# joeyee/Onet

Hardware: AMD Instinct MI355X
Metric: training images/sec (twin 256x256 pass) (higher is better)
Workload: dtype f32

## Files before the change

onet_amd/_lib.py:

```python
from __future__ import annotations

import ctypes
import os
import re

HERE = os.path.dirname(os.path.abspath(__file__))
HEADER = os.path.join(os.path.dirname(HERE), "include", "onet_hip.h")
LIBPATH = os.environ.get("ONET_HIP_LIB") or os.path.join(HERE, "libonet_hip.so")

_CT = {
    "int": ctypes.c_int,
    "int64_t": ctypes.c_int64,
    "uint64_t": ctypes.c_uint64,
    "float": ctypes.c_float,
    "double": ctypes.c_double,
}


def parse_header(path: str = HEADER):
    src = open(path).read()
    src = re.sub(r"/\*.*?\*/", " ", src, flags=re.S)
    src = re.sub(r"//[^\n]*", " ", src)
    src = re.sub(r"^\s*#.*$", " ", src, flags=re.M)
    protos = {}
    for m in re.finditer(r"((?:const\s+)?\w+\s*\*?)\s*(onet_\w+)\s*\(([^)]*)\)\s*;", src):
        ret, name, args = m.group(1).strip(), m.group(2), m.group(3).strip()
        if ret.endswith("*"):
            restype = ctypes.c_char_p if "char" in ret else ctypes.c_void_p
        else:
            restype = _CT[ret]
        argtypes, argnames = [], []
        if args and args != "void":
            for a in args.split(","):
                a = a.strip()
                mm = re.match(r"(?:const\s+)?(\w+)\s*(\*?)\s*(\w+)$", a)
                if not mm:
                    raise ValueError(f"cannot parse argument {a!r} of {name}")
                base, ptr, an = mm.groups()
                argtypes.append(ctypes.c_void_p if ptr else _CT[base])
                argnames.append(an)
        protos[name] = (restype, argtypes, argnames)
    return protos


class OnetHipError(RuntimeError):
    pass


_lib = None
_protos = None


def load(build_if_missing: bool = True):
    global _lib, _protos
    if _lib is not None:
        return _lib
    if not os.path.exists(LIBPATH):
        if not build_if_missing:
            raise OnetHipError(f"{LIBPATH} not built; run `python -m onet_amd.build`")
        from . import build as _build
        _build.build()
    lib = ctypes.CDLL(LIBPATH)
    _protos = parse_header()
    for name, (restype, argtypes, _) in _protos.items():
        try:
            fn = getattr(lib, name)
        except AttributeError as e:
            raise OnetHipError(f"libonet_hip.so does not export {name} declared in onet_hip.h") from e
        fn.restype = restype
        fn.argtypes = argtypes
    _lib = lib
    return lib


def last_error() -> str:
    return load().onet_last_error().decode()


PROFILE_HOOK = None


def call(name: str, *args, nbytes=None):
    lib = load()
    hook = PROFILE_HOOK
    tok = hook.begin() if hook is not None else None
    rc = getattr(lib, name)(*args)
    if tok is not None:
        hook.end(name, nbytes, tok)
    if rc != 0:
        raise OnetHipError(f"{name} failed ({rc}): {lib.onet_last_error().decode()}")
    return rc
```

onet_amd/build.py:

```python
import os
import subprocess
import sys

HERE = os.path.dirname(os.path.abspath(__file__))
CSRC = os.path.join(HERE, "csrc")
LIB = os.path.join(HERE, "libonet_hip.so")
SOURCES = ["abi.cpp", "conv_mfma.hip", "conv_wino4.hip", "conv_wino4w.hip", "conv_split.hip", "convt_gemm.hip", "stem.hip", "bn.hip", "spatial.hip", "head_loss.hip", "optim.hip", "evalside.hip", "clutter.hip"]
ARCH = "gfx950"


def _stale():
    if not os.path.exists(LIB):
        return True
    t = os.path.getmtime(LIB)
    deps = [os.path.join(CSRC, f) for f in os.listdir(CSRC) if f.endswith((".hip", ".cpp", ".hpp"))] + \
        [os.path.join(HERE, "..", "include", "onet_hip.h")]
    return any(os.path.getmtime(d) > t for d in deps)


def build(force=False, verbose=False, variant=None, flags=()):
    lib = LIB if variant is None else os.path.join(HERE, f"libonet_hip_{variant}.so")
    if variant is None and not force and not _stale():
        return LIB
    hipcc = os.environ.get("HIPCC", "/opt/rocm/bin/hipcc")
    objdir = CSRC if variant is None else os.path.join(CSRC, "_" + variant)
    os.makedirs(objdir, exist_ok=True)
    objs = []
    procs = []
    for src in SOURCES:
        obj = os.path.join(objdir, src.rsplit(".", 1)[0] + ".o")
        cmd = [hipcc, "-x", "hip", f"--offload-arch={ARCH}", "-O3", "-fPIC", "-std=c++17", "-Wall",
               "-Wno-unused-result", "-fno-slp-vectorize", *flags, "-c", os.path.join(CSRC, src), "-o", obj]
        if verbose:
            cmd.insert(-4, "-Rpass-analysis=kernel-resource-usage")
        procs.append((src, subprocess.Popen(cmd, stdout=subprocess.PIPE, stderr=subprocess.STDOUT, text=True)))
        objs.append(obj)
    failed = False
    for src, p in procs:
        out, _ = p.communicate()
        if p.returncode != 0:
            failed = True
            sys.stderr.write(f"[onet_amd.build] {src} failed:\n{out}\n")
        elif verbose or out.strip():
            sys.stderr.write(out)
    if failed:
        raise RuntimeError("hipcc failed building libonet_hip.so")
    subprocess.check_call([hipcc, "-shared", "-fPIC", f"--offload-arch={ARCH}", "-o", lib] + objs)
    return lib


if __name__ == "__main__":
    if "--variant" in sys.argv:
        i = sys.argv.index("--variant")
        print(build(variant=sys.argv[i + 1], flags=[a for a in sys.argv[i + 2:]]))
    else:
        print(build(force="--force" in sys.argv, verbose="-v" in sys.argv))
```

onet_amd/csrc/stem.hip:

```cpp
#include <algorithm>
#include "common.hpp"

using namespace onet;

namespace {

struct StemArgs {
    const float* x;
    int64_t x_bs;
    const float* w;
    float* z;
    int64_t z_bs;
    float* part;
    int B, Cout, H, W, tilesX, tilesY;
    int twin_B;
    float twin_bias;
};

constexpr int ST_TH = 16, ST_TW = 64, ST_LR = ST_TH + 2, ST_LC = ST_TW + 4;
constexpr int ST_MAXC = 128;

#define ONET_ST_DPP_ADD(v, ctrl, rmask) \
    v += __builtin_bit_cast(float, __builtin_amdgcn_update_dpp(0, __builtin_bit_cast(int, v), ctrl, rmask, 0xf, false))
__device__ __forceinline__ float wave_sum_hi(float v) {
    ONET_ST_DPP_ADD(v, 0x128, 0xf);
    ONET_ST_DPP_ADD(v, 0x124, 0xf);
    ONET_ST_DPP_ADD(v, 0x122, 0xf);
    ONET_ST_DPP_ADD(v, 0x121, 0xf);
    ONET_ST_DPP_ADD(v, 0x142, 0xa);
    ONET_ST_DPP_ADD(v, 0x143, 0xc);
    return v;
}
#undef ONET_ST_DPP_ADD

template <int CIN>
__global__ __launch_bounds__(256) void stem_conv_stats_kernel(StemArgs a) {
    __shared__ float tile[CIN][ST_LR][ST_LC];
    __shared__ float sc[4][ST_MAXC][2];
    int bid = blockIdx.x;
    const int tx = bid % a.tilesX;
    bid /= a.tilesX;
    const int ty = bid % a.tilesY;
    const int b = bid / a.tilesY;
    const int y0 = ty * ST_TH, x0 = tx * ST_TW;
    const int tid = threadIdx.x, lane = tid & 63, wid = tid >> 6;
    const int HW = a.H * a.W;
    const bool comp = a.twin_B > 0 && b >= a.twin_B;
    const float* xb = a.x + (int64_t)(comp ? b - a.twin_B : b) * a.x_bs;

    for (int i = tid; i < CIN * ST_LR * 66; i += 256) {
        const int ci = i / (ST_LR * 66), r = (i / 66) % ST_LR, c = i % 66;
        const int yy = y0 - 1 + r, xx = x0 - 1 + c;
        const bool ok = yy >= 0 && yy < a.H && xx >= 0 && xx < a.W;
        float v = ok ? xb[(int64_t)ci * HW + (int64_t)yy * a.W + xx] : 0.f;
        if (comp && ok) v = fminf(fmaxf(1.f - v + a.twin_bias, 0.f), 1.f);
        tile[ci][r][c] = v;
    }
    __syncthreads();

    const int r = tid >> 4, q = tid & 15;
    float win[CIN][3][6];
#pragma unroll
    for (int ci = 0; ci < CIN; ++ci)
#pragma unroll
        for (int dy = 0; dy < 3; ++dy)
#pragma unroll
            for (int dx = 0; dx < 6; ++dx) win[ci][dy][dx] = tile[ci][r + dy][4 * q + dx];

    float* zb = a.z + (int64_t)b * a.z_bs + (int64_t)(y0 + r) * a.W + x0 + 4 * q;
    for (int co = 0; co < a.Cout; ++co) {
        const float* wp = a.w + (int64_t)co * CIN * 9;
        float acc[4] = {0.f, 0.f, 0.f, 0.f};
#pragma unroll
        for (int ci = 0; ci < CIN; ++ci)
#pragma unroll
            for (int dy = 0; dy < 3; ++dy)
#pragma unroll
                for (int dx = 0; dx < 3; ++dx) {
                    const float wv = wp[(ci * 3 + dy) * 3 + dx];
#pragma unroll
                    for (int j = 0; j < 4; ++j) acc[j] = fmaf(wv, win[ci][dy][dx + j], acc[j]);
                }
        *reinterpret_cast<float4*>(zb + (int64_t)co * HW) = make_float4(acc[0], acc[1], acc[2], acc[3]);
        if (a.part) {
            const float pv = __builtin_bit_cast(float, __builtin_amdgcn_readfirstlane(__builtin_bit_cast(int, acc[0])));
            float s1 = 0.f, s2 = 0.f;
#pragma unroll
            for (int j = 0; j < 4; ++j) {
                const float d = acc[j] - pv;
                s1 += d;
                s2 = fmaf(d, d, s2);
            }
            s1 = wave_sum_hi(s1);
            s2 = wave_sum_hi(s2);
            if (lane == 63) {
                sc[wid][co][0] = fmaf(s1, 1.f / 256.f, pv);
                sc[wid][co][1] = fmaxf(fmaf(-s1 * (1.f / 256.f), s1, s2), 0.f);
            }
        }
    }
    if (a.part) {
        __syncthreads();
        if (tid < a.Cout) {
            float mw[4], qw[4];
#pragma unroll
            for (int w = 0; w < 4; ++w) {
                mw[w] = sc[w][tid][0];
                qw[w] = sc[w][tid][1];
            }
            const float mean = 0.25f * ((mw[0] + mw[1]) + (mw[2] + mw[3]));
            float m2 = (qw[0] + qw[1]) + (qw[2] + qw[3]);
#pragma unroll
            for (int w = 0; w < 4; ++w) m2 = fmaf(256.f * (mw[w] - mean), mw[w] - mean, m2);
            const int64_t nblk = (int64_t)a.B * a.tilesY * a.tilesX;
            const int64_t blk = ((int64_t)b * a.tilesY + ty) * a.tilesX + tx;
            float* sp = a.part + ((int64_t)tid * nblk + blk) * 3;
            sp[0] = 1024.f;
            sp[1] = mean;
            sp[2] = m2;
        }
    }
}

int stem_nparts(int B, int Cin, int Cout, int H, int W) {
    if (B <= 0 || Cin < 1 || Cin > 4 || Cout < 1 || Cout > ST_MAXC || H <= 0 || W <= 0 || (H % ST_TH) || (W % ST_TW)) return 0;
    const int64_t n = (int64_t)B * (H / ST_TH) * (W / ST_TW);
    return n < (1 << 30) ? (int)n : 0;
}

}

extern "C" {

int onet_conv3x3_stem_nparts(int B, int Cin, int Cout, int H, int W) { return stem_nparts(B, Cin, Cout, H, W); }

int onet_conv3x3_stem_fwd_stats(const float* x, int64_t x_bs, const float* w, float* z, int64_t z_bs, float* part, int B, int Cin,
                                int Cout, int H, int W, int twin_B, float twin_bias, void* stream) {
    ONET_REQUIRE(x && w && z, "conv3x3_stem_fwd_stats: null pointer");
    ONET_REQUIRE(stem_nparts(B, Cin, Cout, H, W) > 0,
                 "conv3x3_stem_fwd_stats: needs 1 <= Cin <= 4, Cout <= %d and a map made of full 16 x 64 tiles (onet_conv3x3_stem_nparts() == 0 elsewhere)",
                 ST_MAXC);
    ONET_REQUIRE(x_bs >= (int64_t)Cin * H * W && z_bs >= (int64_t)Cout * H * W, "conv3x3_stem_fwd_stats: batch stride too small");
    ONET_REQUIRE((z_bs & 3) == 0 && (reinterpret_cast<uintptr_t>(z) & 15) == 0, "conv3x3_stem_fwd_stats: 16-byte aligned output rows required");
    ONET_REQUIRE(twin_B == 0 || 2 * twin_B == B, "conv3x3_stem_fwd_stats: a twin batch holds twin_B = B / 2 images in memory");
    StemArgs a{x, x_bs, w, z, z_bs, part, B, Cout, H, W, W / ST_TW, H / ST_TH, twin_B, twin_bias};
    const int64_t blocks = (int64_t)B * a.tilesX * a.tilesY;
    const dim3 g((unsigned)blocks), t(256);
    switch (Cin) {
        case 1: hipLaunchKernelGGL(stem_conv_stats_kernel<1>, g, t, 0, as_stream(stream), a); break;
        case 2: hipLaunchKernelGGL(stem_conv_stats_kernel<2>, g, t, 0, as_stream(stream), a); break;
        case 3: hipLaunchKernelGGL(stem_conv_stats_kernel<3>, g, t, 0, as_stream(stream), a); break;
        default: hipLaunchKernelGGL(stem_conv_stats_kernel<4>, g, t, 0, as_stream(stream), a); break;
    }
    return check_launch("stem_conv_stats_kernel");
}

}
```

onet_amd/functional.py:

```python
from __future__ import annotations

import torch

from . import ops


def _carries_settings(cls):
    fwd, bwd = cls.forward, cls.backward

    def forward(ctx, *args, **kw):
        ctx._onet_settings = ops.active_settings()
        return fwd(ctx, *args, **kw)

    def backward(ctx, *grads):
        if torch.is_grad_enabled():
            raise RuntimeError("onet_amd: double differentiation (create_graph=True) is not supported: the HIP backward kernels "
                               "build no graph of their own")
        with ops.using(getattr(ctx, "_onet_settings", None)):
            return bwd(ctx, *grads)

    forward.__doc__, backward.__doc__ = fwd.__doc__, bwd.__doc__
    cls.forward, cls.backward = staticmethod(forward), staticmethod(backward)
    return cls

# ... 32 lines not shown
        if norm is not None:
            z, cm = ops.conv3x3_fwd_bn_partials(None, packed, norm=norm)
        else:
            z, cm = ops.conv3x3_fwd_bn_partials(x, packed, amax=x_amax) if training else (ops.conv3x3_auto(x, packed, 0, amax=x_amax), None)
        dst = None if out is None else out[0]
        G = groups if (training and groups > 1) else 1
        C = z.shape[1]
        save_all = torch.empty((G, 4, C), dtype=torch.float32, device=z.device)
        Bz, _, Hz, Wz = z.shape
        pooled = None
        a_amax = ops.new_amax(z.device) if (not defer and z.is_cuda and ops.split_f16() and ops.split_enabled()
                                            and ops.conv_algo() in ("auto", "split", "bf16")) else None
        act_slots = ops.new_amax(z.device) if (defer and ops.split_f16()) else None
        if want_pool is not None and ops.FUSE_POOL and Hz % 2 == 0 and Wz % 4 == 0:
            pooled = (torch.empty((Bz, C, Hz // 2, Wz // 2), dtype=torch.float32, device=z.device), None)

        def apply(zg, sv, o, sl):
            nonlocal pooled
            if defer:
                return None
            if pooled is not None:
                if o is None:
                    o = torch.empty_like(zg)
                if ops.bn_relu_apply_pool(zg, sv, o, pooled[0][sl], amax=a_amax):
                    return o
                pooled = None
            return ops.bn_relu_apply(zg, sv, out=o, amax=a_amax)

        if G == 1:
            if training:
                ops.bn_train_coeffs(z, gamma, beta, running_mean, running_var, momentum, eps,
                                    cm=None if cm is None else (cm, 0, cm.shape[1]), save=save_all[0], act_slots=act_slots)
            else:
                ops.bn_eval_coeffs(gamma, beta, running_mean, running_var, eps, save=save_all[0])
            a = apply(z, save_all[0], dst, slice(0, Bz))
            if defer:
                a = ops.fp32_placeholder(z.shape, z.device)
        else:
            B = z.shape[0]
            Bg = B // G
            a = dst if dst is not None else (ops.fp32_placeholder(z.shape, z.device) if defer else torch.empty_like(z))
            for g in range(G):
                zg = z[g * Bg:(g + 1) * Bg]
                npg = 0 if cm is None else cm.shape[1] // G
                ops.bn_train_coeffs(zg, gamma, beta, running_mean, running_var, momentum, eps,
                                    cm=None if cm is None else (cm, g * npg, npg), save=save_all[g], act_slots=act_slots)
                apply(zg, save_all[g], None if defer else a[g * Bg:(g + 1) * Bg], slice(g * Bg, (g + 1) * Bg))
        if aux is not None:
            aux["a_amax"] = a_amax
        ctx.twin = ops.twin_src_of(x)
        below = (link_in.pop("z"), link_in.pop("save")) if (training and link_in is not None and "z" in link_in) else (None, None)
        ctx.save_for_backward(x, z, save_all, None if norm is None else norm[0], None if norm is None else norm[1], *below)
        ctx.training = training
        ctx.packed = packed
        ctx.wshape = tuple(weight.shape)
        _record_versions(ctx, weight, gamma, beta)
        ctx.link_out = ctx.link_in = None
        if training and link_out is not None:
            link_out.clear()
            link_out.update(z=z, save=save_all)
            if defer:
                link_out["deferred"] = True
                link_out["slots"] = act_slots
            ctx.link_out = link_out
        if below[0] is not None:
            ctx.link_in = link_in
        if pooled is not None and link_out is not None:
            link_out["pooled"] = pooled
        return a

    @staticmethod
    def _forward_pre(ctx, x, weight, gamma, beta, running_mean, running_var, training, momentum, eps, packed, groups, link_out,
                     link_in, p16, aux=None):
        want_pool = link_out.pop("want_pool", None) if link_out is not None else None
        if link_out is not None:
            link_out.pop("defer", None)
        xP = p16.get("x")
        x_slots = p16.get("x_slots") if xP is not None else None
        if xP is not None:
            z, cm = ops.conv3x3_pre_bn_partials(xP, packed, x_slots)
        else:
            x_amax = aux.get("x_amax") if aux is not None else None
            z, cm = ops.conv3x3_fwd_bn_partials(x, packed, amax=x_amax) if training else (ops.conv3x3_auto(x, packed, 0, amax=x_amax), None)
        G = groups if (training and groups > 1) else 1
        Bz, C, Hz, Wz = z.shape
        Bg = Bz // G
        save_all = torch.empty((G, 4, C), dtype=torch.float32, device=z.device)
        want = bool(p16.get("want"))
        keep = bool(p16.get("keep_fp32")) or not want or ops.PRESPLIT_KEEP_FP32
        aP = None
        if want:
            aP = p16.get("out")
            if aP is None:
                aP = ops.p16_empty(Bz, C, Hz, Wz, z.device)
        head = p16.get("head_link")
        defer_head = bool(head is not None and training and G == 2 and not want and want_pool is None and z.dtype == torch.float32
                          and ops.HEAD_NORM and not ops.PRESPLIT_KEEP_FP32)
        a = torch.empty(z.shape, dtype=torch.float32, device=z.device) if (keep and not defer_head) else ops.fp32_placeholder(z.shape, z.device)
        parts2 = ops.p16_parts() == 2
        act_slots = ops.new_amax(z.device) if (want and parts2 and training) else None
        a_amax = ops.new_amax(z.device) if (not want and parts2) else None
        pooled = None
        if want_pool is not None and Hz % 2 == 0 and Wz % 2 == 0:
            if want_pool.get("p16"):
                pooled = (None, None, ops.p16_empty(Bz, C, Hz // 2, Wz // 2, z.device))
            else:
                pooled = (torch.empty((Bz, C, Hz // 2, Wz // 2), dtype=torch.float32, device=z.device), None, None)
        if training and cm is not None:
            ops.bn_train_coeffs(z[:Bg], gamma, beta, running_mean, running_var, momentum, eps, cm=(cm, 0, cm.shape[1] // G), save=save_all,
                                act_slots=act_slots, groups=G)
        else:
            for g in range(G):
                if training:
                    ops.bn_train_coeffs(z[g * Bg:(g + 1) * Bg], gamma, beta, running_mean, running_var, momentum, eps, save=save_all[g],
                                        act_slots=act_slots)
                else:
                    ops.bn_eval_coeffs(gamma, beta, running_mean, running_var, eps, save=save_all[g])
        gi = Bg if G > 1 else 0
        if defer_head:
            head["z"], head["save"] = z, save_all
            head["bwd_fuse"] = xP is not None
            a_amax = None
        elif pooled is not None:
            if not ops.bn_relu_apply_pool_split(z, save_all, aP, a if keep else None, pooled[2], pooled[0], slots=act_slots, group_images=gi):
                raise RuntimeError("onet_amd: pre-split BatchNorm + pooling pass refused a shape ops.pre_layer_ok accepted")
        elif aP is not None:
            ops.bn_relu_apply_split(z, save_all, aP, a=a if keep else None, slots=act_slots, group_images=gi)
        else:
            ops.bn_relu_apply(z, save_all, out=a, amax=a_amax, group_images=gi)
        p16["a"], p16["a_slots"], p16["a_amax"] = aP, act_slots, a_amax
        ctx.x_slots = x_slots
        ctx.up_link = p16.get("up_link")
        ctx.up_want = None if ctx.up_link is None else ctx.up_link.get("want")
        ctx.twin = ops.twin_src_of(x)
        ctx.head_link = head if defer_head else None
        below = (link_in.pop("z"), link_in.pop("save")) if (training and link_in is not None and "z" in link_in) else (None, None)
        ctx.save_for_backward(x, z, save_all, xP, *below)
        ctx.pre = True
        ctx.training = training
        ctx.packed = packed
        ctx.wshape = tuple(weight.shape)
        _record_versions(ctx, weight, gamma, beta)
        ctx.link_out = ctx.link_in = None
        if training and link_out is not None:
            link_out.clear()
            link_out.update(z=z, save=save_all)
            ctx.link_out = link_out
        if below[0] is not None:
            ctx.link_in = link_in
        if pooled is not None and link_out is not None:
            link_out["pooled"] = pooled
        return a

    @staticmethod
    def _retag_twin(ctx, x):
        tw = getattr(ctx, "twin", None)
        if tw is not None and x is not None and ops.twin_src_of(x) is None:
            x._onet_twin_src = [tw[0], tw[1], None]
        return x

    @staticmethod
    def _take_head_handoff(link, da):
        if link is None or "gl" not in link:
            return None
        rda, rec4, da_amax, gl = link.pop("da"), link.pop("rec4"), link.pop("da_amax", None), link.pop("gl")
        if not ops.is_placeholder(da) or rda.data_ptr() != da.data_ptr() or rda.shape != da.shape or rda.stride() != da.stride():
            raise RuntimeError("onet_amd: the head kept the gradient of the last activation unwritten, but autograd handed its unit "
                               "another tensor (a second consumer of that activation?)")
        return rec4, da_amax, gl

    @staticmethod
    def _backward_pre(ctx, da):
        x, z, save_all, xP, z_below, save_below = ctx.saved_tensors
        x = ConvBNReLUFn._retag_twin(ctx, x)
        need_x, need_w, need_g, need_b = ctx.needs_input_grad[:4]
        _check_versions(ctx, (True, True, False))
        pw, pg, pb = ctx.params
        aff = (ops.grad_slot_if_free(pg) if need_g else None, ops.grad_slot_if_free(pb) if need_b else None)
        rec4, da_amax = None, None
        lk = ctx.link_out
        if lk is not None and "rec4" in lk:
            rda, rec4, da_amax = lk.pop("da"), lk.pop("rec4", None), lk.pop("da_amax", None)
            lk.pop("rec", None)
            if rda.data_ptr() != da.data_ptr() or rda.shape != da.shape or rda.stride() != da.stride():
                rec4 = da_amax = None
        da_gl = None
        hand = ConvBNReLUFn._take_head_handoff(getattr(ctx, "head_link", None), da)
        if hand is not None:
            rec4, da_amax, da_gl = hand
        nones = (None,) * 12
        if xP is None:
            if need_w and not need_x and x.shape[1] <= 4 and ops.STEM_WGRAD_BN and (not ops.is_placeholder(x) or ops.twin_src_of(x) is not None):
                dw, dgamma, dbeta = ops.stem_wgrad_bn(x, da, z, save_all, ctx.training, ctx.wshape, affine_out=aff, rec4=rec4,
                                                      out=ops.grad_slot_if_free(pw))
                return (None, dw, (dgamma if need_g else None), (dbeta if need_b else None)) + nones
            dz, dgamma, dbeta = ops.bn_relu_bwd_groups(da, z, save_all, ctx.training, affine_out=aff, rec4=rec4)
            dw = ops.conv3x3_wgrad_auto(x, dz, ctx.wshape, out=ops.grad_slot_if_free(pw)) if need_w else None
            dx = ops.conv3x3_auto(dz, ctx.packed, 1) if need_x else None
            return (dx, dw, (dgamma if need_g else None), (dbeta if need_b else None)) + nones
        dzP, dz_slots, dgamma, dbeta = ops.bn_relu_bwd_split(da, z, save_all, ctx.training, need_affine_grads=(need_g or need_b),
                                                             affine_out=aff, rec4=rec4, da_amax=da_amax, da_gl=da_gl)
        s1, s2, sc = ops._slots3(getattr(ctx, "x_slots", None))
        dw = ops.conv3x3_split_wgrad_pre(xP, dzP, ctx.wshape, out=ops.grad_slot_if_free(pw), x_slots=s1, dz_slots=dz_slots, x_slots2=s2,
                                         split_ch=sc) if need_w else None
        dpack = ctx.packed.get_pack("split" if dzP.shape[3] == 2 else "plain16")[1]
        dx = None
        if need_x and z_below is not None and save_below is not None and ctx.training:
            fused = ops.conv3x3_split_dgrad_pre_bnreduce(dzP, dpack, ctx.wshape[1], z_below, save_below, slots=dz_slots,
# ... 469 lines not shown
```

onet_amd/ops.py:

```python
from __future__ import annotations

import torch

from . import _lib

F32 = torch.float32


import os as _os


def _flags_from_env():
    out = {}
    for item in _os.environ.get("ONET_FLAGS", "").split(","):
        if "=" in item:
            k, v = item.split("=", 1)
            out[k.strip()] = v.strip()
    return out


_FLAGS = _flags_from_env()


def _flag(name, default):
# ... 594 lines not shown
        if B * -(-H // 16) * -(-W // 32) * -(-Cout // 64) >= (n_cu() * 3) // 4:
            return "split"
    if algo == "auto_nosplit":
        algo = "auto"
    if algo == "bf16":
        if Cin % 16 == 0 and Cout % 4 == 0 and W >= 16 and H >= 8:
            return "bf16"
        algo = "auto"
    if algo == "direct" or not _wino_legal(Cin, Cout):
        return "direct"
    if min(H, W) < 8:
        return "direct"
    if algo == "winograd4":
        return "winograd4"
    if min(H, W) >= 16:
        img = 1 if W > 16 else 2
        blocks = -(-B // img) * -(-W // (32 if W > 16 else 16)) * -(-H // 16) * -(-Cout // 64)
        if blocks >= (n_cu() * 7) // 8:
            return "winograd4"
    return "direct"


def use_winograd(Cin, Cout, H, W):
    return conv_algo() != "direct" and _wino_legal(Cin, Cout) and min(H, W) >= 8


class Packed3x3(dict):

    def __init__(self, w):
        super().__init__(Cin=w.shape[1], Cout=w.shape[0])
        self.w = w.detach()

    def get_pack(self, algo):
        if algo not in self:
            self[algo] = {"direct": pack3x3, "winograd4": pack3x3_winograd4, "split": pack3x3_split, "plain16": pack3x3_plain16}[algo](self.w)
        return self[algo]


def pack3x3_auto(w):
    return Packed3x3(w)


def _fp32_algo(B, Cin, Cout, H, W):
    algo = conv3x3_algo(B, Cin, Cout, H, W)
    if algo != "bf16":
        return algo
    cur = active_settings()
    with using(cur.replace(conv="auto") if cur is not None else Settings(conv="auto")):
        return conv3x3_algo(B, Cin, Cout, H, W)


def conv3x3_auto(x, pk, direction, out=None, amax=None):
    Ci, Co = (pk["Cin"], pk["Cout"]) if direction == 0 else (pk["Cout"], pk["Cin"])
    shp = x.shape
    algo = _fp32_algo(shp[0], Ci, Co, shp[2], shp[3])
    if algo == "split" and direction == 1 and not split_dgrad():
        with using(active_settings().replace(split=False) if active_settings() is not None else Settings(split=False)):
            algo = _fp32_algo(shp[0], Ci, Co, shp[2], shp[3])
    wq = pk.get_pack(algo)[direction]
    if algo == "winograd4":
        return conv3x3_winograd4(x, wq, Co, out=out)
    if algo == "split":
        if direction == 0 and amax is None and wq.dtype == torch.float16:
            amax = absmax_slots(x)
        return conv3x3_split(x, wq, Co, out=out, amax=amax, always=direction == 1)
    return conv_fwd(x, wq, Co, 3, out=out)


BN_ON_LOAD = _flag("BN_ON_LOAD", True)
BN_ON_LOAD_MAX_COUT = 128
CONVT_SPLIT_MIN_BLOCKS = None
CONVT_SPLIT = _flag("CONVT_SPLIT", True)
SPLIT_F16 = _flag("SPLIT_F16", True)
SPLIT_DGRAD = _flag("SPLIT_DGRAD", True)
PRESPLIT = _flag("PRESPLIT", True)
PRESPLIT_W16 = _flag("PRESPLIT_W16", True)
PRESPLIT_KEEP_FP32 = _flag("PRESPLIT_KEEP_FP32", False)
SPLIT_GRAD_F16 = _flag("SPLIT_GRAD_F16", False)
SPLIT_WGRAD_MINW = 16
SPLIT_AUTO = _flag("SPLIT", True)
STEM_FUSED = _flag("STEM_FUSED", True)


def conv3x3_fwd_bn_partials(x, pk, norm=None, amax=None):
    Ci, Co = pk["Cin"], pk["Cout"]
    if norm is not None:
        z_prev, save, slots = norm
        require_gpu(z_prev, save)
        zs, zbs = plane(z_prev)
        B, _, H, W = zs.shape
        nparts = int(_lib.load().onet_conv3x3_split_nparts(B, H, W)) if not sync_bn() else 0
        out = torch.empty((B, Co, H, W), dtype=F32, device=zs.device)
        cm = torch.empty((Co, nparts, 3), dtype=F32, device=zs.device) if nparts > 0 else None
        e0 = _prof_begin("conv3x3_split_kernel")
        wq = pk.get_pack("split")[0]
        f16 = wq.dtype == torch.float16
        _lib.call("onet_conv3x3_split_fwd_norm", _p(zs), zbs, _p(save), save.shape[0], _p(wq), int(f16), _p(slots) if f16 else None,
                  _p(out), Co * H * W, _p(cm), B, Ci, Co, H, W, _stream())
        _prof_end("conv3x3_split_kernel", 2.0 * B * H * W * Ci * Co * 9, e0, 4.0 * (B * H * W * (Ci + Co) + 9 * Ci * Co))
        return out, cm
    B, _, H, W = x.shape
    if Ci <= 4 and stem_fused() and not sync_bn() and hasattr(pk, "w"):
        nparts = int(_lib.load().onet_conv3x3_stem_nparts(B, Ci, Co, H, W))
        if nparts > 0:
            require_gpu(x)
            tw = twin_src_of(x)
            xs, xbs = plane(tw[0] if tw is not None else x)
            w = pk.w if pk.w.is_contiguous() else pk.w.contiguous()
            out = torch.empty((B, Co, H, W), dtype=F32, device=x.device)
            cm = torch.empty((Co, nparts, 3), dtype=F32, device=x.device)
            e0 = _prof_begin("stem_conv_stats_kernel")
            _lib.call("onet_conv3x3_stem_fwd_stats", _p(xs), xbs, _p(w), _p(out), Co * H * W, _p(cm), B, Ci, Co, H, W,
                      B // 2 if tw is not None else 0, tw[1] if tw is not None else 0.0, _stream())
            _prof_end("stem_conv_stats_kernel", 2.0 * B * H * W * Ci * Co * 9, e0, 4.0 * (B * H * W * (Ci + Co) + 9 * Ci * Co))
            return out, cm
    algo = _fp32_algo(B, Ci, Co, H, W)
    nparts = 0
    if algo == "winograd4" and not sync_bn():
        nparts = int(_lib.load().onet_conv3x3_winograd4_nparts(B, H, W))
    if algo == "split" and not sync_bn():
        nparts = int(_lib.load().onet_conv3x3_split_nparts(B, H, W))
        if nparts > 0:
            wq = pk.get_pack(algo)[0]
            require_gpu(x)
            xs, xbs = plane(x)
            if xs.data_ptr() % 16 or xbs % 4:
                xs = xs.contiguous()
                xbs = xs.stride(0) if B > 1 else xs[0].numel()
            out = torch.empty((B, Co, H, W), dtype=F32, device=x.device)
            cm = torch.empty((Co, nparts, 3), dtype=F32, device=x.device)
            if wq.dtype == torch.float16 and amax is None:
                amax = absmax_slots(xs)
            e0 = _prof_begin("conv3x3_split_kernel")
            if wq.dtype == torch.float16:
                _lib.call("onet_conv3x3_split_conv_amax", _p(xs), xbs, _p(amax), 0, _p(wq), _p(out), Co * H * W, _p(cm), B, Ci, Co, H, W,
                          _stream())
            else:
                _lib.call("onet_conv3x3_split_fwd_stats", _p(xs), xbs, _p(wq), 0, _p(out), Co * H * W, _p(cm), B, Ci, Co, H, W, _stream())
            _prof_end("conv3x3_split_kernel", 2.0 * B * H * W * Ci * Co * 9, e0, 4.0 * (B * H * W * (Ci + Co) + 9 * Ci * Co))
            return out, cm
    if nparts <= 0:
        return conv3x3_auto(x, pk, 0, amax=amax), None
    wq = pk.get_pack(algo)[0]
    require_gpu(x, wq)
    x, xbs = plane(x)
    out = torch.empty((B, Co, H, W), dtype=F32, device=x.device)
    cm = torch.empty((Co, nparts, 3), dtype=F32, device=x.device)
    e0 = _prof_begin("conv_wino4_kernel")
    _lib.call("onet_conv3x3_winograd4_fwd_stats", _p(x), xbs, _p(wq), _p(out), Co * H * W, _p(cm), B, Ci, Co, H, W,
              _stream())
    _prof_end("conv_wino4_kernel", 2.0 * B * H * W * Ci * Co * 9, e0, 4.0 * (B * H * W * (Ci + Co) + 9 * Ci * Co))
    return out, cm


FUSE_BN_REDUCE = _flag("FUSE_BN_REDUCE", True)


def conv3x3_dgrad_bnreduce(dz, pk, z_prev, save_prev):
    if not FUSE_BN_REDUCE or sync_bn():
        return None
    Ci, Co = pk["Cout"], pk["Cin"]
    B, _, H, W = dz.shape
    if conv3x3_algo(B, Ci, Co, H, W) != "winograd4":
        return None
    nparts = int(_lib.load().onet_conv3x3_winograd4_nparts(B, H, W))
    G = save_prev.shape[0]
    if nparts <= 0 or B % G or tuple(z_prev.shape) != (B, Co, H, W) or not save_prev.is_contiguous():
        return None
    z_prev, zbs = plane(z_prev)
    if (zbs & 3) or (z_prev.data_ptr() & 15):
        return None
    wq = pk.get_pack("winograd4")[1]
    require_gpu(dz, wq, z_prev, save_prev)
    dz, dbs = plane(dz)
    da = torch.empty((B, Co, H, W), dtype=F32, device=dz.device)
    rec = torch.empty((Co, nparts, 2), dtype=F32, device=dz.device)
    e0 = _prof_begin("conv_wino4_kernel")
    _lib.call("onet_conv3x3_winograd4_dgrad_bnreduce", _p(dz), dbs, _p(wq), _p(da), Co * H * W, _p(z_prev), zbs,
              _p(save_prev), B // G, _p(rec), B, Ci, Co, H, W, _stream())
    _prof_end("conv_wino4_kernel", 2.0 * B * H * W * Ci * Co * 9, e0, 4.0 * (B * H * W * (Ci + Co) + 9 * Ci * Co))
    return da, rec






def pack3x3_winograd4(w):
    require_gpu(w)
    w = w.detach().contiguous()
    Cout, Cin = w.shape[0], w.shape[1]
    wf = torch.empty(Cin * 36 * ((Cout + 63) // 64 * 64), dtype=F32, device=w.device)
    wd = torch.empty(Cout * 36 * ((Cin + 63) // 64 * 64), dtype=F32, device=w.device)
    _lib.call("onet_conv3x3_pack_weights_winograd4", _p(w), _p(wf), _p(wd), Cout, Cin, _stream())
    return wf, wd


def conv3x3_winograd4(x, wq, Cout, out=None):
# ... 299 lines not shown
FUSE_DGRAD_REDUCE = _flag("FUSE_DGRAD_REDUCE", True)


def conv3x3_split_wgrad_pre(xs, dzs, dw_shape, out=None, x_slots=None, dz_slots=None, x_slots2=None, split_ch=0):
    if xs.dtype != dzs.dtype or xs.dtype not in (torch.bfloat16, torch.float16):
        raise TypeError("conv3x3_split_wgrad_pre: xs and dzs must be pre-split tensors of the same 16-bit type")
    B, C8, H, two, W, eight = xs.shape
    Cin, Cout = C8 * 8, dzs.shape[1] * 8
    assert tuple(dw_shape) == (Cout, Cin, 3, 3) and dzs.shape[3] == two
    dw = out if out is not None else torch.empty(dw_shape, dtype=F32, device=xs.device)
    need = _lib.load().onet_conv3x3_split_wgrad_ws_bytes(B, Cin, Cout, H, W)
    ws = workspace(need, xs.device)
    e0 = _prof_begin("conv3x3_split_wgrad_pre_kernel")
    _lib.call("onet_conv3x3_split_wgrad_pre", _p(xs), _pbs(xs), _p(x_slots), _p(x_slots2), int(split_ch), _p(dzs),
              _pbs(dzs), _p(dz_slots), 2 if two == 1 else int(xs.dtype == torch.float16), _p(dw), _p(ws),
              ws.numel() * 4, B, Cin, Cout, H, W, 0, _stream())
    _prof_end("conv3x3_split_wgrad_pre_kernel", 2.0 * B * H * W * Cin * Cout * 9, e0,
              2.0 * two * B * H * W * (Cin + Cout) + 4.0 * 9 * Cin * Cout)
    return dw


def pre_layer_ok(B, Cin, Cout, H, W):
    if not presplit() or Cin % 16 or Cout % 16 or W < 16 or (W % 32 and W != 16) or H % 16 or H * W >= 2 ** 24:
        return False
    np_ = p16_parts()
    if np_ == 1 and (Cin % 32 or Cout % 32):
        return False
    if W <= 32 and B * max(Cin, Cout) * H * W * 2 * np_ >= 2 ** 31:
        return False
    lib = _lib.load()
    if W == 16:
        return PRESPLIT_W16 and B % 4 == 0 and (B // 2) * -(-min(Cin, Cout) // 64) >= (n_cu() * 3) // 4 and \
            bool(lib.onet_conv3x3_split_wgrad_pre_ok(B, Cin, Cout, H, W)) and int(lib.onet_maxpool2_bwd_bn_bands(H, W)) >= 0
    want = "bf16" if np_ == 1 else "split"
    return conv3x3_algo(B, Cin, Cout, H, W) == want and conv3x3_algo(B, Cout, Cin, H, W) == want and \
        bool(lib.onet_conv3x3_split_wgrad_pre_ok(B, Cin, Cout, H, W)) and int(lib.onet_conv3x3_split_nparts(B, H, W)) > 0 and \
        int(lib.onet_maxpool2_bwd_bn_bands(H, W)) > 0


def p16_empty(B, C, H, W, device, parts=None):
    parts = p16_parts() if parts is None else parts
    return torch.empty((B, C // 8, H, parts, W, 8), dtype=torch.float16 if parts == 2 else BF, device=device)


def p16_of(t):
    tag = getattr(t, "_onet_p16", None)
    if tag is None:
        return None
    return tag[0] if tag[1] == t._version else None


def p16_slots(t):
    tag = getattr(t, "_onet_p16", None)
    if tag is None or tag[1] != t._version:
        return None
    return tag[2]


def tag_p16(t, P, slots=None):
    if P is not None and t is not None:
        t._onet_p16 = (P, t._version, slots)
    return t


def _slots3(info):
    if isinstance(info, tuple):
        return info
    return info, None, 0


def _pbs(P):
    return P.stride(0) // 2 if P.shape[0] > 1 else P.shape[1] * P.shape[2] * P.shape[3] * P.shape[4] * 4


def bn_relu_apply_split(z, save, xs, a=None, slots=None, group_images=0):
    z, zbs = plane(z)
    B, C, H, W = z.shape
    assert group_images == 0 or (B % group_images == 0 and save.numel() == (B // group_images) * 4 * C and save.is_contiguous())
    _lib.call("onet_bn_relu_apply_split", _p(z), _z16(z), zbs, _p(xs), _pbs(xs), _p(a), 0 if a is None else (a.stride(0) if B > 1 else C * H * W),
              _p(save), _p(slots), xs.shape[3], group_images, B, C, H, W, _stream(),
              nbytes=(z.element_size() + 2 * xs.shape[3] + 4 * (a is not None)) * z.numel())


def bn_relu_apply_pool_split(z, save, xs, a, ys, y, slots=None, group_images=0):
    z, zbs = plane(z)
    B, C, H, W = z.shape
    assert group_images == 0 or (B % group_images == 0 and save.numel() == (B // group_images) * 4 * C and save.is_contiguous())
    n, m = C * H * W, C * (H // 2) * (W // 2)
    rc = _lib.load().onet_bn_relu_apply_pool_split(_p(z), _z16(z), zbs, _p(xs), 0 if xs is None else _pbs(xs), _p(a),
                                                  0 if a is None else (a.stride(0) if B > 1 else n), _p(ys), 0 if ys is None else _pbs(ys),
                                                  _p(y), 0 if y is None else (y.stride(0) if B > 1 else m), _p(save), _p(slots),
                                                  (xs if xs is not None else ys).shape[3] if (xs is not None or ys is not None) else 2,
                                                  group_images, B, C, H, W, _stream())
    if rc < 0:
        raise _lib.OnetHipError(f"onet_bn_relu_apply_pool_split failed ({rc}): {_lib.last_error()}")
    return rc == 0


def conv3x3_pre_bn_partials(xP, pk, slots=None):
    B, C8, H, np_, W, _ = xP.shape
    Co = pk["Cout"]
    wq = pk.get_pack("split" if np_ == 2 else "plain16")[0]
    nparts = int(_lib.load().onet_conv3x3_split_pre_nparts(B, H, W))
    cm = torch.empty((Co, nparts, 3), dtype=F32, device=xP.device) if nparts > 0 else None
    s1, s2, sc = _slots3(slots)
    return conv3x3_split_pre(xP, wq, Co, slots=s1, stats=cm, slots2=s2, split_ch=sc, z16=cm is not None and np_ == 1 and z16_storage()), cm


def _bn_bwd_groups(da, dabs, z, zbs, save_all, training, affine_out, rec4, da_amax, dz_slots):
    B, C, H, W = z.shape
    HW = H * W
    G = save_all.shape[0]
    Bg = B // G
    dev = z.device
    assert B % G == 0 and save_all.is_contiguous()
    if rec4 is None:
        nparts = _bn_nparts(Bg, HW)
        rec4 = torch.empty((G * nparts, C, 4), dtype=F32, device=dev)
        _lib.call("onet_bn_relu_bwd_reduce", _p(da), dabs, _p(z), _z16(z), zbs, _p(save_all), _p(rec4), G * nparts, _p(da_amax), Bg if G > 1 else 0,
                  B, C, HW, _stream(), nbytes=(4 + z.element_size()) * z.numel())
    else:
        assert rec4.shape[0] % G == 0 and rec4.shape[1] == C and rec4.shape[2] == 4 and rec4.is_contiguous()
    og, ob = affine_out if affine_out is not None else (None, None)
    dgamma = torch.empty(C, dtype=F32, device=dev) if og is None else og
    dbeta = torch.empty(C, dtype=F32, device=dev) if ob is None else ob
    coef = torch.empty((G, 4, C), dtype=F32, device=dev) if training else None
    _lib.call("onet_bn_bwd_finalize", _p(rec4), rec4.shape[0] // G, Bg * HW, _p(dgamma), _p(dbeta), _p(coef), 0, G, C, _p(save_all),
              _p(da_amax), _p(dz_slots), _stream())
    return coef, dgamma, dbeta


def bn_relu_bwd_split(da, z, save_all, training, need_affine_grads=True, affine_out=None, rec=None, rec4=None, da_amax=None, da_gl=None):
    if da_gl is not None:
        if rec4 is None or _z16(z) or (p16_parts() == 2 and da_amax is None):
            raise RuntimeError("onet_amd: a BatchNorm backward on an unmaterialised g * L needs the records of the fused head backward")
        gmap = da_gl[0]
        da, dabs = plane(da_gl[1])
        assert gmap.is_contiguous() and gmap.shape[0] == z.shape[0] and gmap.numel() == z.shape[0] * z.shape[2] * z.shape[3] and da.shape == z.shape
    else:
        da, dabs = plane(da)
    z, zbs = plane(z)
    B, C, H, W = z.shape
    G = save_all.shape[0]
    dev = z.device
    np_ = p16_parts()
    dzP = p16_empty(B, C, H, W, dev, np_)
    scaled = np_ == 2
    dz_slots = new_amax(dev) if scaled else None
    if scaled and rec4 is not None and da_amax is None:
        da_amax = absmax_slots(da)
    if rec4 is None:
        da_amax = new_amax(dev) if scaled else None
    coef, dgamma, dbeta = _bn_bwd_groups(da, dabs, z, zbs, save_all, training, affine_out, rec4, da_amax, dz_slots)
    if da_gl is not None:
        _lib.call("onet_bn_relu_bwd_apply_split_gl", _p(da), dabs, _p(gmap), _p(z), zbs, _p(save_all), _p(coef), _p(dzP), _pbs(dzP), _p(dz_slots), np_,
                  B // G if G > 1 else 0, B, C, H, W, _stream(), nbytes=(8 + 2 * np_) * z.numel() + 4 * gmap.numel())
        return dzP, dz_slots, dgamma, dbeta
    _lib.call("onet_bn_relu_bwd_apply_split", _p(da), dabs, _p(z), _z16(z), zbs, _p(save_all), _p(coef), _p(dzP), _pbs(dzP), _p(dz_slots), np_,
              B // G if G > 1 else 0, B, C, H, W, _stream(), nbytes=(4 + z.element_size() + 2 * np_) * z.numel())
    return dzP, dz_slots, dgamma, dbeta


def stem_wgrad_bn(x, da, z, save_all, training, dw_shape, affine_out=None, rec4=None, out=None, twin=None):
    require_gpu(x, da, z)
    if twin is None:
        twin = twin_src_of(x)
    B, Cin, H, W = x.shape
    x, xbs = plane(twin[0] if twin is not None else x)
    da, dabs = plane(da)
    z, zbs = plane(z)
    Cout = z.shape[1]
    G = save_all.shape[0]
    coef, dgamma, dbeta = _bn_bwd_groups(da, dabs, z, zbs, save_all, training, affine_out, rec4, None, None)
    dw = torch.empty(dw_shape, dtype=F32, device=x.device) if out is None else out
    ws = workspace(_lib.load().onet_conv_wgrad_ws_bytes(B, Cin, Cout, H, W, 3), x.device)
    e0 = _prof_begin("conv_wgrad_kernel")
    _lib.call("onet_conv3x3_stem_wgrad_bn", _p(x), xbs, _p(da), dabs, _p(z), zbs, _p(save_all), _p(coef), B // G if G > 1 else 0, _p(dw),
              _p(ws), ws.numel() * 4, B, Cin, Cout, H, W, 0, B // 2 if twin is not None else 0, twin[1] if twin is not None else 0.0, _stream())
    _prof_end("conv_wgrad_kernel", 2.0 * B * H * W * Cin * Cout * 9, e0, 4.0 * (B * H * W * (Cin + 2 * Cout) + 9 * Cin * Cout))
    return dw, dgamma, dbeta


STEM_WGRAD_BN = _flag("STEM_WGRAD_BN", True)


def bn_relu_bwd_groups(da, z, save_all, training, affine_out=None, rec4=None):
    da, dabs = plane(da)
    z, zbs = plane(z)
    B, C, H, W = z.shape
    G = save_all.shape[0]
    coef, dgamma, dbeta = _bn_bwd_groups(da, dabs, z, zbs, save_all, training, affine_out, rec4, None, None)
    dz = torch.empty((B, C, H, W), dtype=F32, device=z.device)
    _lib.call("onet_bn_relu_bwd_apply", _p(da), dabs, _p(z), zbs, _p(save_all), _p(coef), _p(dz), C * H * W, None, B // G if G > 1 else 0,
              B, C, H * W, _stream(), nbytes=12 * z.numel())
    return dz, dgamma, dbeta


def split_wgrad_ok(x, dz):
    B, Cin, H, W = x.shape
    ok = bool(_lib.load().onet_conv3x3_split_wgrad_ok(B, Cin, dz.shape[1], H, W)) and \
        x.stride(0) % 4 == 0 and x.data_ptr() % 16 == 0 and dz.is_contiguous() and dz.data_ptr() % 16 == 0 and \
        max(Cin, dz.shape[1]) * H * W * 4 < 2 ** 31
    if ok and W < 64:
        ok = ((B - 1) * x.stride(0) + Cin * H * W) * 4 < 2 ** 31 and B * dz.shape[1] * H * W * 4 < 2 ** 31
    return ok


def norm_on_load_ok(B, Cmid, Cout, H, W, groups):
    if not _setting("bn_on_load", BN_ON_LOAD) or sync_bn() or conv_algo() not in ("auto", "split") or groups not in (1, 2) or B % groups:
        return False
    if conv3x3_algo(B, Cmid, Cout, H, W) != "split" or W < SPLIT_WGRAD_MINW:
        return False
    if Cout > BN_ON_LOAD_MAX_COUT:
        return False
    if not _lib.load().onet_conv3x3_split_wgrad_ok(B, Cmid, Cout, H, W) or max(Cmid, Cout) * H * W * 4 >= 2 ** 31:
        return False
    return W >= 64 or B * max(Cmid, Cout) * H * W * 4 < 2 ** 31


def conv3x3_split_wgrad(x, dz, dw_shape, out=None, norm=None, dz_amax=None, x_amax=None):
    if dz_amax is not None:
        require_gpu(x, dz)
        x, xbs = plane(x)
        dz, dzbs = plane(dz)
        B, Cin, H, W = x.shape
        Cout = dz.shape[1]
        dw = torch.empty(dw_shape, dtype=F32, device=x.device) if out is None else out
        ws = workspace(_lib.load().onet_conv3x3_split_wgrad_ws_bytes(B, Cin, Cout, H, W), x.device)
        e0 = _prof_begin("conv3x3_split_wgrad_kernel")
        _lib.call("onet_conv3x3_split_wgrad_f16", _p(x), xbs, _p(x_amax), _p(norm), 0 if norm is None else norm.shape[0], _p(dz), dzbs,
                  _p(dz_amax), _p(dw), _p(ws), ws.numel() * 4, B, Cin, Cout, H, W, 0, _stream())
        _prof_end("conv3x3_split_wgrad_kernel", 2.0 * B * H * W * Cin * Cout * 9, e0, 4.0 * (B * H * W * (Cin + Cout) + 9 * Cin * Cout))
        return dw
    if norm is not None:
        require_gpu(x, dz, norm)
        x, xbs = plane(x)
        dz, dzbs = plane(dz)
        B, Cin, H, W = x.shape
        Cout = dz.shape[1]
        dw = torch.empty(dw_shape, dtype=F32, device=x.device) if out is None else out
        ws = workspace(_lib.load().onet_conv3x3_split_wgrad_ws_bytes(B, Cin, Cout, H, W), x.device)
        e0 = _prof_begin("conv3x3_split_wgrad_kernel")
        _lib.call("onet_conv3x3_split_wgrad_norm", _p(x), xbs, _p(norm), norm.shape[0], _p(dz), dzbs, _p(dw), _p(ws), ws.numel() * 4,
                  B, Cin, Cout, H, W, 0, _stream())
        _prof_end("conv3x3_split_wgrad_kernel", 2.0 * B * H * W * Cin * Cout * 9, e0, 4.0 * (B * H * W * (Cin + Cout) + 9 * Cin * Cout))
        return dw
    require_gpu(x, dz)
    x, xbs = plane(x)
    dz, dzbs = plane(dz)
    B, Cin, H, W = x.shape
    Cout = dz.shape[1]
    dw = torch.empty(dw_shape, dtype=F32, device=x.device) if out is None else out
    need = _lib.load().onet_conv3x3_split_wgrad_ws_bytes(B, Cin, Cout, H, W)
    ws = workspace(need, x.device)
    e0 = _prof_begin("conv3x3_split_wgrad_kernel")
    _lib.call("onet_conv3x3_split_wgrad", _p(x), xbs, _p(dz), dzbs, _p(dw), _p(ws), ws.numel() * 4, B, Cin, Cout, H, W, 0, _stream())
    _prof_end("conv3x3_split_wgrad_kernel", 2.0 * B * H * W * Cin * Cout * 9, e0, 4.0 * (B * H * W * (Cin + Cout) + 9 * Cin * Cout))
    return dw


def _engine_accumulates(param):
    try:
        return bool(torch._C._will_engine_execute_node(torch.autograd.graph.get_gradient_edge(param).node))
    except RuntimeError:
        return False

# ... 578 lines not shown
```

Baseline: 598.0.

## Recompute stem conv inside the BN+ReLU split-apply pass instead of reading z

Adds a stem_apply_split kernel that recomputes the cheap low-Cin 3x3 stem convolution from the input tile, applies BatchNorm+ReLU, and writes the two-part split activation directly. This removes the read of the full fp32 stem output z in the apply pass, trading it for redundant conv arithmetic. Enabled by default in training when the stem path applies and z is not kept.

```diff
diff --git a/include/onet_hip_stem.h b/include/onet_hip_stem.h
--- /dev/null
+++ b/include/onet_hip_stem.h
@@ -0,0 +1,15 @@
+#ifndef ONET_HIP_STEM_H
+#define ONET_HIP_STEM_H
+#include <stdint.h>
+#ifdef __cplusplus
+extern "C" {
+#endif
+
+int onet_conv3x3_stem_apply_split(const float* x, int64_t x_bs, const float* w, const float* save, void* xs, int64_t xs_bs,
+                                  const void* act_amax, int group_images, int B, int Cin, int Cout, int H, int W, int twin_B, float twin_bias,
+                                  void* stream);
+
+#ifdef __cplusplus
+}
+#endif
+#endif
diff --git a/onet_amd/_lib.py b/onet_amd/_lib.py
--- a/onet_amd/_lib.py
+++ b/onet_amd/_lib.py
@@ -6,6 +6,7 @@
 
 HERE = os.path.dirname(os.path.abspath(__file__))
 HEADER = os.path.join(os.path.dirname(HERE), "include", "onet_hip.h")
+MORE_HEADERS = [os.path.join(os.path.dirname(HERE), "include", "onet_hip_stem.h")]
 LIBPATH = os.environ.get("ONET_HIP_LIB") or os.path.join(HERE, "libonet_hip.so")
 
 _CT = {
@@ -62,6 +63,8 @@
         _build.build()
     lib = ctypes.CDLL(LIBPATH)
     _protos = parse_header()
+    for h in MORE_HEADERS:
+        _protos.update(parse_header(h))
     for name, (restype, argtypes, _) in _protos.items():
         try:
             fn = getattr(lib, name)
diff --git a/onet_amd/build.py b/onet_amd/build.py
--- a/onet_amd/build.py
+++ b/onet_amd/build.py
@@ -14,7 +14,7 @@
         return True
     t = os.path.getmtime(LIB)
     deps = [os.path.join(CSRC, f) for f in os.listdir(CSRC) if f.endswith((".hip", ".cpp", ".hpp"))] + \
-        [os.path.join(HERE, "..", "include", "onet_hip.h")]
+        [os.path.join(HERE, "..", "include", h) for h in ("onet_hip.h", "onet_hip_stem.h")]
     return any(os.path.getmtime(d) > t for d in deps)
 
 
diff --git a/onet_amd/csrc/stem.hip b/onet_amd/csrc/stem.hip
--- a/onet_amd/csrc/stem.hip
+++ b/onet_amd/csrc/stem.hip
@@ -1,5 +1,6 @@
 #include <algorithm>
 #include "common.hpp"
+#include "../../include/onet_hip_stem.h"
 
 using namespace onet;
 
@@ -32,6 +33,37 @@
     return v;
 }
 #undef ONET_ST_DPP_ADD
+
+template <int CIN, int ST = 1, int WN>
+__device__ __forceinline__ void stem_conv_z4(const float* wp, const float (&win)[CIN][3][WN], float (&acc)[4]) {
+    static_assert(WN >= 3 * ST + 3, "window too narrow");
+#pragma unroll
+    for (int j = 0; j < 4; ++j) acc[j] = 0.f;
+#pragma unroll
+    for (int ci = 0; ci < CIN; ++ci)
+#pragma unroll
+        for (int dy = 0; dy < 3; ++dy)
+#pragma unroll
+            for (int dx = 0; dx < 3; ++dx) {
+                const float wv = wp[(ci * 3 + dy) * 3 + dx];
+#pragma unroll
+                for (int j = 0; j < 4; ++j) acc[j] = fmaf(wv, win[ci][dy][dx + ST * j], acc[j]);
+            }
+}
+
+template <int CIN>
+__device__ __forceinline__ void stem_fill_tile(float (&tile)[CIN][ST_LR][ST_LC], const float* xb, bool comp, float twin_bias, int y0, int x0,
+                                               int H, int W) {
+    const int HW = H * W;
+    for (int i = threadIdx.x; i < CIN * ST_LR * 66; i += 256) {
+        const int ci = i / (ST_LR * 66), r = (i / 66) % ST_LR, c = i % 66;
+        const int yy = y0 - 1 + r, xx = x0 - 1 + c;
+        const bool ok = yy >= 0 && yy < H && xx >= 0 && xx < W;
+        float v = ok ? xb[(int64_t)ci * HW + (int64_t)yy * W + xx] : 0.f;
+        if (comp && ok) v = fminf(fmaxf(1.f - v + twin_bias, 0.f), 1.f);
+        tile[ci][r][c] = v;
+    }
+}
 
 template <int CIN>
 __global__ __launch_bounds__(256) void stem_conv_stats_kernel(StemArgs a) {
@@ -48,14 +80,7 @@
     const bool comp = a.twin_B > 0 && b >= a.twin_B;
     const float* xb = a.x + (int64_t)(comp ? b - a.twin_B : b) * a.x_bs;
 
-    for (int i = tid; i < CIN * ST_LR * 66; i += 256) {
-        const int ci = i / (ST_LR * 66), r = (i / 66) % ST_LR, c = i % 66;
-        const int yy = y0 - 1 + r, xx = x0 - 1 + c;
-        const bool ok = yy >= 0 && yy < a.H && xx >= 0 && xx < a.W;
-        float v = ok ? xb[(int64_t)ci * HW + (int64_t)yy * a.W + xx] : 0.f;
-        if (comp && ok) v = fminf(fmaxf(1.f - v + a.twin_bias, 0.f), 1.f);
-        tile[ci][r][c] = v;
-    }
+    stem_fill_tile<CIN>(tile, xb, comp, a.twin_bias, y0, x0, a.H, a.W);
     __syncthreads();
 
     const int r = tid >> 4, q = tid & 15;
@@ -70,17 +95,8 @@
     float* zb = a.z + (int64_t)b * a.z_bs + (int64_t)(y0 + r) * a.W + x0 + 4 * q;
     for (int co = 0; co < a.Cout; ++co) {
         const float* wp = a.w + (int64_t)co * CIN * 9;
-        float acc[4] = {0.f, 0.f, 0.f, 0.f};
-#pragma unroll
-        for (int ci = 0; ci < CIN; ++ci)
-#pragma unroll
-            for (int dy = 0; dy < 3; ++dy)
-#pragma unroll
-                for (int dx = 0; dx < 3; ++dx) {
-                    const float wv = wp[(ci * 3 + dy) * 3 + dx];
-#pragma unroll
-                    for (int j = 0; j < 4; ++j) acc[j] = fmaf(wv, win[ci][dy][dx + j], acc[j]);
-                }
+        float acc[4];
+        stem_conv_z4<CIN>(wp, win, acc);
         *reinterpret_cast<float4*>(zb + (int64_t)co * HW) = make_float4(acc[0], acc[1], acc[2], acc[3]);
         if (a.part) {
             const float pv = __builtin_bit_cast(float, __builtin_amdgcn_readfirstlane(__builtin_bit_cast(int, acc[0])));
@@ -118,6 +134,76 @@
             sp[0] = 1024.f;
             sp[1] = mean;
             sp[2] = m2;
+        }
+    }
+}
+
+struct StemApplyArgs {
+    const float* x;
+    int64_t x_bs;
+    const float* w;
+    const float* save;
+    unsigned* xs;
+    int64_t xs_bs;
+    const unsigned* slots;
+    int B, Cout, H, W, tilesX, tilesY, gimg, twin_B;
+    float twin_bias;
+};
+typedef unsigned st_u32x4 __attribute__((ext_vector_type(4)));
+
+template <int CIN>
+__global__ __launch_bounds__(256) void stem_apply_split_kernel(StemApplyArgs a) {
+    __shared__ float tile[CIN][ST_LR][ST_LC];
+    float s_inv;
+    const float s_act = amax_scale(amax_read(a.slots), false, s_inv);
+    int bid = blockIdx.x;
+    const int tx = bid % a.tilesX;
+    bid /= a.tilesX;
+    const int ty = bid % a.tilesY;
+    const int b = bid / a.tilesY;
+    const int y0 = ty * ST_TH, x0 = tx * ST_TW;
+    const int tid = threadIdx.x;
+    const bool comp = a.twin_B > 0 && b >= a.twin_B;
+    stem_fill_tile<CIN>(tile, a.x + (int64_t)(comp ? b - a.twin_B : b) * a.x_bs, comp, a.twin_bias, y0, x0, a.H, a.W);
+    __syncthreads();
+
+    const int r = tid >> 4, q = tid & 15;
+    float win[CIN][3][12];
+#pragma unroll
+    for (int ci = 0; ci < CIN; ++ci)
+#pragma unroll
+        for (int dy = 0; dy < 3; ++dy)
+#pragma unroll
+            for (int j = 0; j < 4; ++j)
+#pragma unroll
+                for (int dx = 0; dx < 3; ++dx) win[ci][dy][3 * j + dx] = tile[ci][r + dy][q + 16 * j + dx];
+
+    const float* sv = a.save + (a.gimg ? (int64_t)(b / a.gimg) * 4 * a.Cout : 0);
+    st_u32x4* const dst = reinterpret_cast<st_u32x4*>(a.xs + (int64_t)b * a.xs_bs);
+    for (int c8 = 0; c8 < (a.Cout >> 3); ++c8) {
+        float v[4][8];
+#pragma unroll
+        for (int k = 0; k < 8; ++k) {
+            const int c = c8 * 8 + k;
+            const float mean = sv[c], sc = sv[2 * a.Cout + c], sh = sv[3 * a.Cout + c];
+            float z[4];
+            stem_conv_z4<CIN, 3>(a.w + (int64_t)c * CIN * 9, win, z);
+#pragma unroll
+            for (int j = 0; j < 4; ++j) v[j][k] = fmaxf(fmaf(z[j] - mean, sc, sh), 0.f);
+        }
+        const int64_t row = ((int64_t)(c8 * a.H + y0 + r) * 2) * a.W + x0 + q;
+#pragma unroll
+        for (int j = 0; j < 4; ++j) {
+            st_u32x4 hi, mid;
+#pragma unroll
+            for (int k = 0; k < 4; ++k) {
+                unsigned h, m;
+                split2h_s(v[j][2 * k], v[j][2 * k + 1], s_act, h, m);
+                hi[k] = h;
+                mid[k] = m;
+            }
+            dst[row + 16 * j] = hi;
+            dst[row + a.W + 16 * j] = mid;
         }
     }
 }
@@ -155,4 +241,26 @@
     return check_launch("stem_conv_stats_kernel");
 }
 
-}
+int onet_conv3x3_stem_apply_split(const float* x, int64_t x_bs, const float* w, const float* save, void* xs, int64_t xs_bs,
+                                  const void* act_amax, int group_images, int B, int Cin, int Cout, int H, int W, int twin_B, float twin_bias,
+                                  void* stream) {
+    ONET_REQUIRE(x && w && save && xs && group_images >= 0, "conv3x3_stem_apply_split: bad args");
+    ONET_REQUIRE(stem_nparts(B, Cin, Cout, H, W) > 0 && (Cout % 8) == 0,
+                 "conv3x3_stem_apply_split: needs the stem kernel's shapes (onet_conv3x3_stem_nparts() > 0) and Cout %% 8 == 0");
+    ONET_REQUIRE(x_bs >= (int64_t)Cin * H * W && xs_bs >= (int64_t)Cout * H * W && (xs_bs & 3) == 0 && (reinterpret_cast<uintptr_t>(xs) & 15) == 0,
+                 "conv3x3_stem_apply_split: batch stride too small or slots not 16-byte aligned");
+    ONET_REQUIRE(twin_B == 0 || 2 * twin_B == B, "conv3x3_stem_apply_split: a twin batch holds twin_B = B / 2 images in memory");
+    ONET_REQUIRE(group_images == 0 || B % group_images == 0, "conv3x3_stem_apply_split: B must be a multiple of group_images");
+    StemApplyArgs a{x, x_bs, w, save, (unsigned*)xs, xs_bs, (const unsigned*)act_amax, B, Cout, H, W, W / ST_TW, H / ST_TH, group_images, twin_B,
+                    twin_bias};
+    const dim3 g((unsigned)((int64_t)B * a.tilesX * a.tilesY)), t(256);
+    switch (Cin) {
+        case 1: hipLaunchKernelGGL(stem_apply_split_kernel<1>, g, t, 0, as_stream(stream), a); break;
+        case 2: hipLaunchKernelGGL(stem_apply_split_kernel<2>, g, t, 0, as_stream(stream), a); break;
+        case 3: hipLaunchKernelGGL(stem_apply_split_kernel<3>, g, t, 0, as_stream(stream), a); break;
+        default: hipLaunchKernelGGL(stem_apply_split_kernel<4>, g, t, 0, as_stream(stream), a); break;
+    }
+    return check_launch("stem_apply_split_kernel");
+}
+
+}
diff --git a/onet_amd/functional.py b/onet_amd/functional.py
--- a/onet_amd/functional.py
+++ b/onet_amd/functional.py
@@ -138,6 +138,7 @@
         else:
             x_amax = aux.get("x_amax") if aux is not None else None
             z, cm = ops.conv3x3_fwd_bn_partials(x, packed, amax=x_amax) if training else (ops.conv3x3_auto(x, packed, 0, amax=x_amax), None)
+        stem_z = bool(training and xP is None and ops.stem_fwd_ok(x, packed))
         G = groups if (training and groups > 1) else 1
         Bz, C, Hz, Wz = z.shape
         Bg = Bz // G
@@ -180,6 +181,8 @@
         elif pooled is not None:
             if not ops.bn_relu_apply_pool_split(z, save_all, aP, a if keep else None, pooled[2], pooled[0], slots=act_slots, group_images=gi):
                 raise RuntimeError("onet_amd: pre-split BatchNorm + pooling pass refused a shape ops.pre_layer_ok accepted")
+        elif aP is not None and not keep and stem_z and ops.STEM_APPLY_RECOMPUTE and aP.shape[3] == 2 and C % 8 == 0:
+            ops.stem_apply_split(x, packed, save_all, aP, slots=act_slots, group_images=gi)
         elif aP is not None:
             ops.bn_relu_apply_split(z, save_all, aP, a=a if keep else None, slots=act_slots, group_images=gi)
         else:
diff --git a/onet_amd/ops.py b/onet_amd/ops.py
--- a/onet_amd/ops.py
+++ b/onet_amd/ops.py
@@ -700,6 +700,12 @@
 STEM_FUSED = _flag("STEM_FUSED", True)
 
 
+def stem_fwd_ok(x, pk):
+    B, _, H, W = x.shape
+    Ci, Co = pk["Cin"], pk["Cout"]
+    return Ci <= 4 and stem_fused() and not sync_bn() and hasattr(pk, "w") and int(_lib.load().onet_conv3x3_stem_nparts(B, Ci, Co, H, W)) > 0
+
+
 def conv3x3_fwd_bn_partials(x, pk, norm=None, amax=None):
     Ci, Co = pk["Cin"], pk["Cout"]
     if norm is not None:
@@ -718,20 +724,19 @@
         _prof_end("conv3x3_split_kernel", 2.0 * B * H * W * Ci * Co * 9, e0, 4.0 * (B * H * W * (Ci + Co) + 9 * Ci * Co))
         return out, cm
     B, _, H, W = x.shape
-    if Ci <= 4 and stem_fused() and not sync_bn() and hasattr(pk, "w"):
+    if stem_fwd_ok(x, pk):
         nparts = int(_lib.load().onet_conv3x3_stem_nparts(B, Ci, Co, H, W))
-        if nparts > 0:
-            require_gpu(x)
-            tw = twin_src_of(x)
-            xs, xbs = plane(tw[0] if tw is not None else x)
-            w = pk.w if pk.w.is_contiguous() else pk.w.contiguous()
-            out = torch.empty((B, Co, H, W), dtype=F32, device=x.device)
-            cm = torch.empty((Co, nparts, 3), dtype=F32, device=x.device)
-            e0 = _prof_begin("stem_conv_stats_kernel")
-            _lib.call("onet_conv3x3_stem_fwd_stats", _p(xs), xbs, _p(w), _p(out), Co * H * W, _p(cm), B, Ci, Co, H, W,
-                      B // 2 if tw is not None else 0, tw[1] if tw is not None else 0.0, _stream())
-            _prof_end("stem_conv_stats_kernel", 2.0 * B * H * W * Ci * Co * 9, e0, 4.0 * (B * H * W * (Ci + Co) + 9 * Ci * Co))
-            return out, cm
+        require_gpu(x)
+        tw = twin_src_of(x)
+        xs, xbs = plane(tw[0] if tw is not None else x)
+        w = pk.w if pk.w.is_contiguous() else pk.w.contiguous()
+        out = torch.empty((B, Co, H, W), dtype=F32, device=x.device)
+        cm = torch.empty((Co, nparts, 3), dtype=F32, device=x.device)
+        e0 = _prof_begin("stem_conv_stats_kernel")
+        _lib.call("onet_conv3x3_stem_fwd_stats", _p(xs), xbs, _p(w), _p(out), Co * H * W, _p(cm), B, Ci, Co, H, W,
+                  B // 2 if tw is not None else 0, tw[1] if tw is not None else 0.0, _stream())
+        _prof_end("stem_conv_stats_kernel", 2.0 * B * H * W * Ci * Co * 9, e0, 4.0 * (B * H * W * (Ci + Co) + 9 * Ci * Co))
+        return out, cm
     algo = _fp32_algo(B, Ci, Co, H, W)
     nparts = 0
     if algo == "winograd4" and not sync_bn():
@@ -1197,6 +1202,19 @@
               nbytes=(z.element_size() + 2 * xs.shape[3] + 4 * (a is not None)) * z.numel())
 
 
+def stem_apply_split(x, pk, save, xs, slots=None, group_images=0):
+    require_gpu(x)
+    B, Ci, H, W = x.shape
+    Co = pk["Cout"]
+    assert xs.shape[3] == 2 and stem_fwd_ok(x, pk)
+    assert group_images == 0 or (B % group_images == 0 and save.numel() == (B // group_images) * 4 * Co and save.is_contiguous())
+    tw = twin_src_of(x)
+    xs_, xbs = plane(tw[0] if tw is not None else x)
+    w = pk.w if pk.w.is_contiguous() else pk.w.contiguous()
+    _lib.call("onet_conv3x3_stem_apply_split", _p(xs_), xbs, _p(w), _p(save), _p(xs), _pbs(xs), _p(slots), group_images, B, Ci, Co, H, W,
+              B // 2 if tw is not None else 0, tw[1] if tw is not None else 0.0, _stream(), nbytes=4 * B * Co * H * W + 4 * x.numel())
+
+
 def bn_relu_apply_pool_split(z, save, xs, a, ys, y, slots=None, group_images=0):
     z, zbs = plane(z)
     B, C, H, W = z.shape
@@ -1297,6 +1315,7 @@
 
 
 STEM_WGRAD_BN = _flag("STEM_WGRAD_BN", True)
+STEM_APPLY_RECOMPUTE = _flag("STEM_APPLY_RECOMPUTE", True)
 
 
 def bn_relu_bwd_groups(da, z, save_all, training, affine_out=None, rec4=None):
```

Result: no change. 601.0, median of 6 (+0.5%).
